# leducthanhig/image-restoration-models

Hardware: AMD Instinct MI355X
Metric: images/sec + PSNR, Restormer motion-deblur 1280x720 (higher is better)
Workload: dtype f32 (1x1 convs: fp32 emulated by 3 fp16 MFMAs on hi/lo operand splits with fp32 accumulation, error vs float64 at the level of an fp32 chain; everything else exact f32; value_exact_f32: f32 MFMA everywhere); 1 GPU; Restormer motion-deblur (WithBias LN, 26.13M params, synthetic weights seed 42) on 1280x720x3 uint8 GoPro-shaped synthetic frames; 6 tiles 512x512 (overlap 96) per frame; a step = 4 frame(s) per GPU, their 24 tiles in one batched forward; global_batch=4, tile=512, overlap=96, parallelism=per-image shard x1, no data-path collective

## Files before the change

image-restoration-models_amd/_hip.py:

```python
from __future__ import annotations

import ctypes as C
import os

import torch

_HERE = os.path.dirname(os.path.abspath(__file__))
LIB_PATH = os.path.join(_HERE, "libirm_hip.so")

ACT_NONE, ACT_RELU, ACT_GELU, ACT_SILU, ACT_RELU6 = 0, 1, 2, 3, 4
LN_NONE, LN_WITHBIAS, LN_BIASFREE = 0, 1, 2

_P, _L, _I, _F, _D = C.c_void_p, C.c_long, C.c_int, C.c_float, C.c_double

SIGNATURES = {
    "irm_version": [],
    "irm_ln_stats_f32": [_P, _L, _P, _I, _I, _I, _F, _P],
    "irm_gemm1x1_f32": [_P, _L, _P, _L, _P, _L, _P, _L, _P, _P, _P, _P, _I, _I, _I, _I, _I, _I, _I, _I, _P, _F, _P, _P],
    "irm_gemm1x1_f16x3_f32": [_P, _L, _P, _L, _P, _L, _P, _L, _P, _P, _P, _P, _I, _I, _I, _I, _I, _I, _I, _I, _P, _F, _P, _P],
    "irm_ln_split_f16": [_P, _L, _P, _P, _I, _F, _F, _P, _I, _I, _I, _P],
    "irm_ln_gemm_presplit_f16x3_f32": [_P, _P, _L, _P, _P, _I, _F, _F, _P, _L, _P, _F, _I, _I, _I, _I, _I, _P],
    "irm_ln_gemm_presplit_cl_f16x3_f32": [_P, _P, _L, _P, _P, _I, _F, _F, _P, _L, _P, _F, _I, _I, _I, _I, _I, _I, _P],
    "irm_gdfn_tail_f16x3_f32": [_P, _L, _P, _P, _P, _P, _L, _F, _I, _I, _I, _I, _I, _I, _P],
    "irm_gemm_presplit_f16x3_f32": [_P, _P, _P, _L, _P, _F, _I, _I, _I, _I, _I, _I, _I, _I, _P],
# ... 40 lines not shown
}

SIGNATURES_HALF = {
    "irm_conv3x3_h_in_f32": [_P, _P, _L, _P, _L, _P, _I, _I, _I, _I, _I, _I, _P],
    "irm_conv3x3_h_f16": [_P, _F, _P, _L, _P, _L, _P, _L, _P, _I, _I, _I, _I, _I, _I, _I, _I, _P],
    "irm_conv3x3_h_out_f32": [_P, _P, _L, _P, _L, _P, _L, _P, _I, _I, _I, _I, _I, _I, _P],
}

SIGNATURES_FRAMES = {
    "irm_frame_minmax_f32": [_P, _L, _P, _P, _L, _P],
    "irm_tile_extract_f32": [_P, _P, _P, _P, _P, _I, _I, _I, _I, _I, _I, _I, _I, _I, _P],
    "irm_window_blend_f32": [_P, _P, _P, _P, _P, _I, _I, _I, _I, _I, _I, _I, _I, _I, _I, _I, _P],
}

SIGNATURES_GRAM = {
    "irm_dw_gram_cm_f16x3_f32": [_P, _L, _P, _P, _P, _P, _I, _I, _I, _I, _I, _P],
}

SIGNATURES_YUV = {
    "irm_yuv420_to_rgb_f32": [_P, _P, _P, _I, _L, _L, _I, _I, _I, _I, _I, _I, _I, _I, _P, _P],
    "irm_rgb_f32_to_yuv420": [_P, _P, _P, _P, _I, _L, _L, _I, _I, _I, _I, _I, _I, _I, _I, _P],
}

SIGNATURES_INCEPTION = {
    "irm_convkxk_f32": [_P, _P, _L, _P, _L, _P, _L, _P, _I, _I, _I, _I, _I, _I, _I, _I, _I, _I, _I, _I, _I, _I, _I, _P],
    "irm_pool3x3_f32": [_P, _L, _P, _L, _I, _I, _I, _I, _I, _P],
}

SIGNATURES_METRICS = {
    "irm_frame_metrics_f32": [_P, _P, _I, _I, _I, _I, _D, _P, _P, _P, _L, _P],
    "irm_yuv420_metrics": [_P, _P, _P, _I, _L, _L, _P, _P, _P, _I, _L, _L, _I, _I, _I, _I, _I, _P, _P, _P, _L, _P],
}

_lib = None


class HipLibraryError(RuntimeError):
    pass


def load():
    global _lib, LIB_PATH
    if _lib is None:
        if os.environ.get("IRM_HIP_LIB"):
            LIB_PATH = os.path.abspath(os.environ["IRM_HIP_LIB"])
        if not os.path.exists(LIB_PATH):
            raise HipLibraryError(
                f"{LIB_PATH} not found: build it with `python -c 'import __graft_entry__ as g; g.build()'` "
                "(make -C image-restoration-models_amd/csrc).  There is no CPU fallback.")
        lib = C.CDLL(LIB_PATH)
        for name, argtypes in {**SIGNATURES, **SIGNATURES_HALF, **SIGNATURES_FRAMES, **SIGNATURES_GRAM,
                               **SIGNATURES_YUV, **SIGNATURES_INCEPTION, **SIGNATURES_METRICS}.items():
            fn = getattr(lib, name)
            fn.argtypes = argtypes
            fn.restype = _I
        _lib = lib
    return _lib


def _stream() -> int:
    return torch.cuda.current_stream().cuda_stream


def ptr(t):
    if t is None:
        return None
    if isinstance(t, int):
        return t
    assert t.is_cuda, "HIP kernels need device tensors"
    return t.data_ptr()


def call(name: str, *args):
    rc = getattr(load(), name)(*args, _stream())
    if rc != 0:
        raise HipLibraryError(f"{name} failed with status {rc} "
                              f"({'invalid arguments' if rc == -1 else 'HIP launch error'})")



def pack_gemm_weight(w: torch.Tensor) -> torch.Tensor:
    w = w.detach().reshape(w.shape[0], -1).float()
    m, k = w.shape
    mt, ks = (m + 15) // 16, 4 * ((k + 15) // 16)
    wpad = torch.zeros(mt * 16, ks * 4, dtype=torch.float32, device=w.device)
# ... 420 lines not shown
```

image-restoration-models_amd/csrc/conv3x3_f16.hip:

```cpp
#include "conv_epilogue.h"


#define CF_TH 8
#define CF_TW IRM_CONV_TW
#define CF_PLANE 400
#define CF_HC 34
#define CF_NP 340
#define CF_PXB 160
#define CF_RAWB (7 * 512 * 16)
#define CF_IMGB (CF_NP * CF_PXB)
#define CF_NRAW 7


__device__ __forceinline__ float cf_res(float v, float r, int mode) {
    if (mode == 1) return v + r;
    if (mode == 2) return r - v;
    return fminf(fmaxf(tanhf(v) + r, -1.0f), 1.0f);
}

struct ConvF16Args {
    const float* Wp;
    const float* X; long x_bs;
    float* Y; long y_bs;
    const float* R; long r_bs;
    const float* bias;
    int Ci, Co, H, W, mtiles, S;
    int relu1, res_mode, relu2, store_mode, tiles_x;
    float inv_s;
    float slope;
    int ps_r;
};


template <int CT, int NCH = 1>
__global__ __launch_bounds__(512, 2) void conv3x3_f16x3_kernel(ConvF16Args a) {
    constexpr int TT = CT * NCH;
    constexpr int NG = 3 * NCH;
    constexpr int WGB = 3 * CT * 2048;
    constexpr int NW = (WGB / 16 + 511) / 512;
    extern __shared__ __attribute__((aligned(16))) float smem[];
    char* lds = reinterpret_cast<char*>(smem);
    char* raw = lds;
    char* img = lds + CF_RAWB;
    char* wbuf = img + CF_IMGB;

    const int tid = threadIdx.x, lane = tid & 63, wave = __builtin_amdgcn_readfirstlane(tid >> 6);
    const int g = lane >> 4, r = lane & 15;
    const int b = blockIdx.z;
    const int ty0 = (blockIdx.x / a.tiles_x) * CF_TH, tx0 = (blockIdx.x % a.tiles_x) * CF_TW;
    const float* X = a.X + (long)b * a.x_bs;
    const long plane = (long)a.H * a.W;
    const int S = a.S;
    const int nchunks = (a.mtiles + TT - 1) / TT;
    const int my_chunks = (nchunks - (int)blockIdx.y + (int)gridDim.y - 1) / (int)gridDim.y;

    long xoff[CF_NRAW];
    int xch[CF_NRAW];
    bool xok[CF_NRAW];
#pragma unroll
    for (int j = 0; j < CF_NRAW; ++j) {
        const int q = j * 512 + tid;
        const int ch = q / 100, rem = q - ch * 100, row = rem / 10, chunk = rem - row * 10;
        const int gy = ty0 - 1 + row, gx = tx0 - 4 + chunk * 4;
        xch[j] = ch;
        xok[j] = q < 3200 && gy >= 0 && gy < a.H && gx >= 0 && gx < a.W;
        xoff[j] = (long)ch * plane + (long)gy * a.W + gx;
    }
    const float* const zero_page = irm_zero_page;
// ... 78 lines not shown
                        const int pi = (wave + dy) * CF_HC + 16 * p + r + dx;
                        ah[p] = *reinterpret_cast<const irm_h8*>(img + pi * CF_PXB + 16 * g);
                        al[p] = *reinterpret_cast<const irm_h8*>(img + pi * CF_PXB + 64 + 16 * g);
                    }
#pragma unroll
                    for (int c = 0; c < CT; ++c) {
                        const irm_h8 wh = *reinterpret_cast<const irm_h8*>(wb + ((c * 3 + tl) * 2) * 1024 + lane * 16);
                        const irm_h8 wl = *reinterpret_cast<const irm_h8*>(wb + ((c * 3 + tl) * 2 + 1) * 1024 + lane * 16);
#pragma unroll
                        for (int p = 0; p < 2; ++p) {
                            f32x4& t = acc[p][chn * CT + c];
                            t = irm_mfma3_f16(ah[p], al[p], wh, wl, t);
                        }
                    }
                }
            }
        }
#pragma unroll
        for (int c = 0; c < TT; ++c) {
            const int co = (mt0 + c) * 16 + r;
            const bool row_ok = mt0 + c < a.mtiles && co < a.Co;
            const float bv = (a.bias && row_ok) ? a.bias[co] : 0.0f;
#pragma unroll
            for (int p = 0; p < 2; ++p) {
                const int y = ty0 + wave, x = tx0 + p * 16 + g * 4;
                float v[4];
#pragma unroll
                for (int e = 0; e < 4; ++e) {
                    v[e] = fmaf(acc[p][c][e], a.inv_s, bv);
                    if (a.relu1 == 1) v[e] = fmaxf(v[e], 0.0f);
                    else if (a.relu1 == 2) v[e] = v[e] > 0.0f ? v[e] : v[e] * a.slope;
                }
                if (!row_ok || y >= a.H || x >= a.W) continue;
                if (a.store_mode == 0) {
                    const long off = (long)co * plane + (long)y * a.W + x;
                    if (a.res_mode) {
                        const float4 rr = *reinterpret_cast<const float4*>(R + off);
                        const float rv[4] = {rr.x, rr.y, rr.z, rr.w};
#pragma unroll
                        for (int e = 0; e < 4; ++e) v[e] = cf_res(v[e], rv[e], a.res_mode);
                    }
                    if (a.relu2) {
#pragma unroll
                        for (int e = 0; e < 4; ++e) v[e] = fmaxf(v[e], 0.0f);
                    }
                    *reinterpret_cast<float4*>(Y + off) = make_float4(v[0], v[1], v[2], v[3]);
                } else if (a.store_mode == 1) {
                    const int oh = a.H >> 1, ow = a.W >> 1;
                    const long op = (long)oh * ow;
                    const int oc = co * 4 + (y & 1) * 2;
                    const long o = (long)(y >> 1) * ow + (x >> 1);
                    *reinterpret_cast<float2*>(Y + (long)oc * op + o) = make_float2(v[0], v[2]);
                    *reinterpret_cast<float2*>(Y + (long)(oc + 1) * op + o) = make_float2(v[1], v[3]);
                } else if (a.ps_r == 2) {
                    const int ow = a.W * 2;
                    const long op = (long)a.H * 2 * ow;
                    const int oc = co >> 2, i = (co >> 1) & 1, jx = co & 1;
                    float* o = Y + (long)oc * op + (long)(2 * y + i) * ow + 2 * x + jx;
#pragma unroll
                    for (int e = 0; e < 4; ++e) o[2 * e] = v[e];
                } else {
                    const int pr = a.ps_r, ow = a.W * pr;
                    const long op = (long)a.H * pr * ow;
                    const int oc = co / (pr * pr), i = (co / pr) % pr, jx = co % pr;
                    float* o = Y + (long)oc * op + (long)(pr * y + i) * ow + pr * x + jx;
#pragma unroll
                    for (int e = 0; e < 4; ++e) o[pr * e] = v[e];
                }
            }
        }
    }
}

template <int CT, int NCH = 1>
static int launch_conv_f16(const ConvF16Args& a, int B, int ygroups, hipStream_t stream) {
    const size_t lds = (size_t)CF_RAWB + CF_IMGB + 2 * (3 * CT * 2048);
    static_assert((size_t)CF_RAWB + CF_IMGB + 2 * (3 * CT * 2048) <= 160 * 1024, "LDS");
    IRM_ALLOW_BIG_LDS((&conv3x3_f16x3_kernel<CT, NCH>));
    const int tiles_y = (a.H + CF_TH - 1) / CF_TH;
    dim3 grid(a.tiles_x * tiles_y, ygroups, B);
    hipLaunchKernelGGL((conv3x3_f16x3_kernel<CT, NCH>), grid, dim3(512), lds, stream, a);
    return irm_launch_status();
}

extern "C" int irm_conv3x3_f16x3_ep_f32(const float* wp_split, float inv_scale, const float* x, long x_bs, float* y,
                                        long y_bs, const float* res, long r_bs, const float* bias, int B, int Ci, int Co,
                                        int H, int W, int act1, float slope, int res_mode, int relu2, int store_mode,
                                        int shuffle, int ct, int ygroups, hipStream_t stream) {
    ConvF16Args a;
    if (int rc = irm_conv_common(a, wp_split, x, x_bs, y, y_bs, res, r_bs, bias, B, Ci, Co, H, W, act1, slope, res_mode,
                                 relu2, store_mode, shuffle, ct, ygroups)) return rc;
    if ((W & 3) || (x_bs & 3) || (y_bs & 3) || (r_bs & 3)) return IRM_EINVAL;
    if (!irm_aligned16(x) || !irm_aligned16(y) || !irm_aligned16(res) || !irm_aligned16(wp_split)) return IRM_EINVAL;
    a.S = (Ci + 31) / 32; a.inv_s = inv_scale;
    switch (ct) {
        case 1: return launch_conv_f16<1>(a, B, ygroups, stream);
        case 2: return launch_conv_f16<2>(a, B, ygroups, stream);
        case 3: return launch_conv_f16<3>(a, B, ygroups, stream);
        case 4: return launch_conv_f16<4>(a, B, ygroups, stream);
        case 8: return launch_conv_f16<4, 2>(a, B, ygroups, stream);
        case 12: return launch_conv_f16<4, 3>(a, B, ygroups, stream);
        default: return IRM_EINVAL;
    }
}

extern "C" int irm_conv3x3_f16x3_f32(const float* wp_split, float inv_scale, const float* x, long x_bs, float* y, long y_bs,
                                     const float* res, long r_bs, const float* bias, int B, int Ci, int Co, int H, int W,
                                     int relu1, int res_mode, int relu2, int store_mode, int ct, int ygroups,
                                     hipStream_t stream) {
    return irm_conv3x3_f16x3_ep_f32(wp_split, inv_scale, x, x_bs, y, y_bs, res, r_bs, bias, B, Ci, Co, H, W, relu1 ? 1 : 0,
                                    0.0f, res_mode, relu2, store_mode, 2, ct, ygroups, stream);
}
```

image-restoration-models_amd/csrc/elementwise.hip:

```cpp
#include "irm_common.h"

template <bool VEC, int PQ>
__global__ __launch_bounds__(256) void ln_stats_kernel(const float* __restrict__ x, long x_bs,
                                                       float* __restrict__ stats, int C, int N, float eps) {
    constexpr int G = 256 / PQ;
    __shared__ float4 pm[G][PQ], pq[G][PQ], ps[G][PQ];
    const int b = blockIdx.y;
    const int q = threadIdx.x % PQ, g = threadIdx.x / PQ;
    const int n = (blockIdx.x * PQ + q) * 4;
    const float* p = x + (long)b * x_bs;
    float4 mean = make_float4(0.f, 0.f, 0.f, 0.f), m2 = mean, sum = mean;
    int cnt = 0;
    auto push = [&](const float4& v) {
        sum.x += v.x; sum.y += v.y; sum.z += v.z; sum.w += v.w;
        const float rc = 1.0f / (float)(++cnt);
        float d;
        d = v.x - mean.x; mean.x += d * rc; m2.x += d * (v.x - mean.x);
        d = v.y - mean.y; mean.y += d * rc; m2.y += d * (v.y - mean.y);
        d = v.z - mean.z; mean.z += d * rc; m2.z += d * (v.z - mean.z);
        d = v.w - mean.w; mean.w += d * rc; m2.w += d * (v.w - mean.w);
    };
    if (n < N) {
        int c = g;
        for (; c + 3 * G < C; c += 4 * G) {
// ... 180 lines not shown
#pragma unroll
        for (int i = 0; i < 6; ++i) { a0[i] = a1[i]; a1[i] = a2[i]; }
    }
}

static int dw_launch(bool gate, const DwArgs& a, int B, hipStream_t stream) {
    constexpr int RS = 8;
    const long total = (long)a.C * ((a.H + RS - 1) / RS) * ((a.W + 3) >> 2);
    const long blocks = (total + 255) / 256;
    if (blocks > 2147483647L || B > 65535) return IRM_EINVAL;
    dim3 grid((unsigned)blocks, B);
    const bool vec = !(a.W & 3) && !(a.x_bs & 3) && !(a.y_bs & 3) && irm_aligned16(a.x) && irm_aligned16(a.y);
    if (gate && vec) hipLaunchKernelGGL((dwconv3x3_kernel<true, RS, true>), grid, dim3(256), 0, stream, a);
    else if (gate) hipLaunchKernelGGL((dwconv3x3_kernel<true, RS, false>), grid, dim3(256), 0, stream, a);
    else if (vec) hipLaunchKernelGGL((dwconv3x3_kernel<false, RS, true>), grid, dim3(256), 0, stream, a);
    else hipLaunchKernelGGL((dwconv3x3_kernel<false, RS, false>), grid, dim3(256), 0, stream, a);
    return irm_launch_status();
}

extern "C" int irm_dwconv3x3_f32(const float* x, long x_bs, const float* w, const float* bias, float* y,
                                 long y_bs, int B, int C, int H, int W, int act, hipStream_t stream) {
    if (!x || !w || !y || B <= 0 || C <= 0 || H <= 0 || W <= 0) return IRM_EINVAL;
    if (act < 0 || act > 3) return IRM_EINVAL;
    DwArgs a{x, x_bs, w, bias, y, y_bs, C, H, W, act};
    return dw_launch(false, a, B, stream);
}

extern "C" int irm_dwconv3x3_gate_f32(const float* x, long x_bs, const float* w, const float* bias, float* y,
                                      long y_bs, int B, int hid, int H, int W, hipStream_t stream) {
    if (!x || !w || !y || B <= 0 || hid <= 0 || H <= 0 || W <= 0) return IRM_EINVAL;
    DwArgs a{x, x_bs, w, bias, y, y_bs, hid, H, W, IRM_ACT_NONE};
    return dw_launch(true, a, B, stream);
}
```

image-restoration-models_amd/ops.py:

```python
from __future__ import annotations

import os

import torch

from . import _hip
from ._hip import ACT_GELU, ACT_NONE, ACT_RELU, ACT_RELU6, ACT_SILU, LN_BIASFREE, LN_NONE, LN_WITHBIAS


class KernelTimer:

    def __init__(self, detail=False, only=None):
        self.records = []
        self.detail = detail
        self.only = None if only is None else frozenset(only)
        self._chain = {}
        self._done = {}
        self._since = 0

    def _fold(self, k, e0, e1, fl, by):
        d = self._done.setdefault(k, dict(launches=0, ms=0.0, flops=0.0, bytes=0.0))
        d["launches"] += 1
        d["ms"] += e0.elapsed_time(e1)
        d["flops"] += fl
# ... 407 lines not shown
        ygroups = max(1, min(nchunks, -(-target_blocks() // blocks)))
    return ct, ygroups


def conv3x3(wp, x, y, ci: int, co: int, *, bias=None, relu1=False, res=None, res_mode=0, relu2=False,
            store_mode=0, ct: int | None = None, ygroups: int | None = None, leaky: float | None = None, shuffle: int = 2):
    _chk(x, "x"), _chk(y, "y")
    B, _, H, W = x.shape
    nbytes = 4.0 * B * H * W * (ci + co + (co if res is not None else 0))
    if leaky is not None and relu1:
        raise ValueError("conv3x3: relu1 and leaky are exclusive")
    act1, slope = (2, float(leaky)) if leaky is not None else (int(bool(relu1)), 0.0)
    extra = (f" ps{shuffle}" if shuffle != 2 else "") + (f" leaky{slope:g}" if leaky is not None else "")
    if isinstance(wp, _hip.ConvWeight):
        aligned = (W % 4 == 0 and _bs(x) % 4 == 0 and _bs(y) % 4 == 0 and _bs(res) % 4 == 0 and x.data_ptr() % 16 == 0
                   and y.data_ptr() % 16 == 0 and (res is None or res.data_ptr() % 16 == 0))
        if wp.raw is not None and aligned and store_mode == 0 and act1 < 2:
            _launch("conv3x3_thin", 18.0 * B * ci * co * H * W, nbytes, "irm_conv3x3_thin_f32", _hip.ptr(wp.raw), _hip.ptr(x),
                    _bs(x), _hip.ptr(y), _bs(y), _hip.ptr(res), _bs(res), _hip.ptr(bias), B, ci, co, H, W, int(relu1),
                    int(res_mode), int(relu2), tag=f"ci{ci} co{co} {H}x{W} B{B}")
            return
        wp = (wp.split, wp.inv_scale) if (wp.split is not None and aligned) else wp.exact
    if isinstance(wp, tuple):
        kernel, entry, lead = "conv3x3_f16x3", "irm_conv3x3_f16x3_ep_f32", (_hip.ptr(wp[0]), float(wp[1]))
    else:
        kernel, entry, lead = "conv3x3", "irm_conv3x3_ep_f32", (_hip.ptr(wp),)
    ct, ygroups = plan_conv3x3(co, H, W, B, split=isinstance(wp, tuple), ct=ct, ygroups=ygroups)
    _launch(kernel, 18.0 * B * ci * co * H * W, nbytes, entry, *lead, _hip.ptr(x), _bs(x), _hip.ptr(y), _bs(y),
            _hip.ptr(res), _bs(res), _hip.ptr(bias), B, ci, co, H, W, act1, slope, int(res_mode), int(relu2),
            int(store_mode), int(shuffle), ct, ygroups,
            tag=f"ci{ci} co{co} {H}x{W} B{B} ct{ct} yg{ygroups} st{store_mode}{extra}")


def transpose(src: torch.Tensor, dst: torch.Tensor, R: int, C: int):
    B = src.shape[0]
    _launch("transpose", 0.0, 8.0 * B * R * C, "irm_transpose_f32", _hip.ptr(src), src.stride(0), _hip.ptr(dst),
            dst.stride(0), B, R, C, tag=f"R{R} C{C} B{B}")


def scan_is_flat(D: int, N: int, R: int) -> bool:
    return (N, R) in ((1, 4), (16, 4)) and D % 64 != 0


def scan_plan(B: int, L: int, D: int, flat: bool = False):
    DB = (D + 63) // 64
    waves = -(-4 * D // 64) if flat else 4 * DB
    nchunk = max(1, min(-(-L // 32), -(-3072 // (B * waves))))
    chunk = max(32, -(-(-(-L // nchunk)) // 8) * 8)
    return chunk, -(-L // chunk), DB


def selective_scan(xT, pT, ids, dtw, dtb, A, Dskip, yT, state, sdt, ysum, B, L, D, N, R, chunk):
    flops = B * 4.0 * L * D * (2 * R + 9 * N + 12)
    nbytes = 4.0 * B * L * (D + 4 * (R + 2 * N) + 4 * D)
    _launch("selective_scan", flops, nbytes, "irm_selective_scan_f32", _hip.ptr(xT), _hip.ptr(pT), _hip.ptr(ids),
            _hip.ptr(dtw), _hip.ptr(dtb), _hip.ptr(A), _hip.ptr(Dskip), _hip.ptr(yT), _hip.ptr(state), _hip.ptr(sdt),
            _hip.ptr(ysum), B, L, D, N, R, chunk, tag=f"L{L} D{D} N{N} B{B} chunk{chunk}")


def losh_combine(ysum, gw, gb, gate, yT, nw, nb, z, out, B, L, D, nchunk, eps=1e-5):
    _chk(z, "z"), _chk(out, "out")
    _launch("losh_combine", 12.0 * B * L * D, 4.0 * B * L * D * 6, "irm_losh_combine_f32", _hip.ptr(ysum), _hip.ptr(gw),
            _hip.ptr(gb), _hip.ptr(gate), _hip.ptr(yT), _hip.ptr(nw), _hip.ptr(nb), _hip.ptr(z), _bs(z), _hip.ptr(out),
            _bs(out), B, L, D, nchunk, float(eps), tag=f"L{L} D{D} B{B}")


# ... 62 lines not shown
```

image-restoration-models_amd/restormer/restormer.py:

```python
from __future__ import annotations

import os

import torch
import torch.nn as nn

from .. import _hip, ops, unet
from ..host import ModelHost, f32

SYNTH_RULES = (
    (r"^output\.weight$", "gain", 0.02),
    (r"^skip_conv\.weight$", "gain", 0.5),
)


def _hidden(dim, factor):
    return int(dim * factor)


class _Norm(nn.Module):

    def __init__(self, dim, kind):
        super().__init__()
        self.body = nn.Module()
# ... 118 lines not shown

    def __init__(self, inp_channels=3, out_channels=3, dim=48, num_blocks=(4, 6, 6, 8),
                 num_refinement_blocks=4, heads=(1, 2, 4, 8), ffn_expansion_factor=2.66, bias=False,
                 LayerNorm_type="WithBias", dual_pixel_task=False):
        super().__init__()
        f, ln = ffn_expansion_factor, LayerNorm_type
        d1, d2, d3, d4 = dim, dim * 2, dim * 4, dim * 8
        self.inp_channels, self.out_channels, self.dim = inp_channels, out_channels, dim
        self.patch_embed = _Proj(inp_channels, d1, bias=False)
        self.encoder_level1 = _stage(d1, heads[0], num_blocks[0], f, bias, ln)
        self.down1_2 = _Resample(d1, d1 // 2)
        self.encoder_level2 = _stage(d2, heads[1], num_blocks[1], f, bias, ln)
        self.down2_3 = _Resample(d2, d2 // 2)
        self.encoder_level3 = _stage(d3, heads[2], num_blocks[2], f, bias, ln)
        self.down3_4 = _Resample(d3, d3 // 2)
        self.latent = _stage(d4, heads[3], num_blocks[3], f, bias, ln)
        self.up4_3 = _Resample(d4, d4 * 2)
        self.reduce_chan_level3 = nn.Conv2d(d4, d3, 1, bias=bias)
        self.decoder_level3 = _stage(d3, heads[2], num_blocks[2], f, bias, ln)
        self.up3_2 = _Resample(d3, d3 * 2)
        self.reduce_chan_level2 = nn.Conv2d(d3, d2, 1, bias=bias)
        self.decoder_level2 = _stage(d2, heads[1], num_blocks[1], f, bias, ln)
        self.up2_1 = _Resample(d2, d2 * 2)
        self.decoder_level1 = _stage(d2, heads[0], num_blocks[0], f, bias, ln)
        self.refinement = _stage(d2, heads[0], num_refinement_blocks, f, bias, ln)
        self.dual_pixel_task = dual_pixel_task
        if dual_pixel_task:
            self.skip_conv = nn.Conv2d(d1, d2, 1, bias=bias)
        self.output = nn.Conv2d(d2, out_channels, 3, padding=1, bias=bias)
        self._split = False
        self.max_tiles_per_batch = 12
        self.hip_graph = True
        self._tap = None

    def _build(self):
        self._split = not os.environ.get("IRM_GEMM_EXACT")
        pk = {name: pack_block(m, self._split) for name, m in self.named_modules() if isinstance(m, TransformerBlock)}
        pk.update(unet.pack_unet(self))
        for name in ("reduce_chan_level3", "reduce_chan_level2"):
            if self._split and _hip.split_is_safe(getattr(self, name).weight):
                pk[name + "_s"] = _hip.pack_gemm_weight_split(getattr(self, name).weight)
        return pk

    def _block(self, blk: TransformerBlock, w: dict, x: torch.Tensor, have_stats: bool = False,
               want_stats: bool = True) -> bool:
        B, C, H, W = x.shape
        N = H * W
        dev = x.device
        heads = blk.attn.num_heads
        hid = blk.ffn.hidden
        fuse = ops.can_fuse_stats(C)
        stats = self._buf("stats", B * 2 * N, dev)
        big_a = self._buf("scratch_a", B * max(3 * C, 2 * hid) * N, dev)
        big_b = self._buf("scratch_b", B * max(3 * C, hid) * N, dev)
        qkv = big_a[:B * 3 * C * N].view(B, 3 * C, H, W)
        qkv2 = big_b[:B * 3 * C * N].view(B, 3 * C, H, W)
        split = self._split and N % 4 == 0
        s_qkv, s_pin, s_pout = split and "qkv_s" in w, split and "pin_s" in w, split and "pout_s" in w
        s_fold = split and w.get("mfold_split", False)
        presplit = split and "qkv_ps" in w and ops.can_presplit(C, N)
        if presplit:
            xs = self._buf("xsplit", B * C * N, dev)
            frag, out_scale, s_x = w["qkv_ps"]
            ops.ln_gemm_presplit(frag, x, qkv, 3 * C, C, w["n1w"], w["n1b"], blk.norm1.mode, s_x, out_scale=out_scale,
                                 bias=w["qkv_b"], xs=xs)
        else:
# ... 59 lines not shown
        N = H * W
        dev = x.device
        heads, hid = blk.attn.num_heads, blk.ffn.hidden
        qkv = self._buf("scratch_a", B * 3 * C * N, dev).view(B, 3 * C, H, W)
        tm = ops.can_qk_tile_major(C, heads, H, W)
        fa = "gdfn_fa" in w
        assert not (x_tm or y_tm) or (tm and fa), "tile-major x / y: only between the kernels that understand them"
        v_tm = tm and fa
        gram_in_qkv = tm and "gram_s" in w and ops.can_qkv_gram(C, heads, H, W)
        nchunk, rec = ops.gram_part_plan(B, C, heads, H, W, tiled=gram_in_qkv)
        nready = None
        part = self._buf("gram_part", B * heads * nchunk * rec, dev)
        if gram_in_qkv:
            nready = ops.qkv_gram_cm(w["qkv_f"], x, qkv, w["gram_s"], part, C, ln_mode=blk.norm1.mode, x_tm=x_tm, v_tm=v_tm)
        else:
            ops.qkv_dw_fused(w["qkv_f"], x, qkv, C, 3 * C, ln_mode=blk.norm1.mode, tm=tm, x_tm=x_tm, v_tm=v_tm)
        gsum = self._buf("gram_sum", B * heads * rec, dev)
        mfold_n = ops.mfold_numel(C)
        mfold = self._zeros(("mfold", C, B), B * mfold_n, dev)
        s_fold = w.get("mfold_split", False)
        if fa:
            mfrag = self._zeros(("mfold_frag", C, B), B * ops.mfold_frag_numel(C), dev)
            ops.mdta_fold(qkv, part, gsum, w["temp"], w["wout"], mfrag, C, heads, gram_scale=w.get("gram_s"), frag=True, tm=tm,
                          nchunk_ready=nready)
            ops.attn_gdfn_fused(w["gdfn_fa"], x, qkv[:, 2 * C:], mfrag, alt, C, hid, ln_mode=blk.norm2.mode,
                                bias_o=w["wout_b"], bias=w["pout_b"], x_tm=x_tm, v_tm=v_tm, y_tm=y_tm)
            return alt
        ops.mdta_fold(qkv, part, gsum, w["temp"], w["wout"], mfold, C, heads, split=s_fold, gram_scale=w.get("gram_s"), tm=tm,
                      nchunk_ready=nready)
        ops.gemm1x1(mfold, qkv[:, 2 * C:], x, C, C, res=x, bias=w["wout_b"], w_bs=mfold_n, split=s_fold)
        ops.gdfn_fused(w["gdfn_f"], x, alt, C, hid, ln_mode=blk.norm2.mode, bias=w["pout_b"])
        return alt

    def _run_stage(self, name, pk, x, have_stats=False):
        names = (name,) if isinstance(name, str) else tuple(name)
        blocks = [(f"{n}.{i}", blk) for n in names for i, blk in enumerate(getattr(self, n))]
        B, C, H, W = x.shape
        if (len(blocks) and all("gdfn_f" in pk[k] for k, _ in blocks) and ops.can_fuse_gdfn(C, W) and (H * W) % 4 == 0
                and len({blk.attn.num_heads for _, blk in blocks}) == 1):
            cur, alt = x, self._buf(f"alt_{C}", B * C * H * W, x.device).view(B, C, H, W)
            heads = blocks[0][1].attn.num_heads
            act_tm = all("gdfn_fa" in pk[k] for k, _ in blocks) and ops.can_qk_tile_major(C, heads, H, W)
            for i, (k, blk) in enumerate(blocks):
                out = self._block_fused(blk, pk[k], cur, alt, x_tm=act_tm and i > 0, y_tm=act_tm and i + 1 < len(blocks))
                cur, alt = out, cur
            if cur is not x:
                x.copy_(cur)
                if ops.TIMER is not None:
                    ops.TIMER.break_chain()
            return False
        for n in names:
            stage = getattr(self, n)
            for i, blk in enumerate(stage):
                have_stats = self._block(blk, pk[f"{n}.{i}"], x, have_stats, want_stats=i + 1 < len(stage))
        return have_stats

    @torch.no_grad()
    def forward(self, inp_img: torch.Tensor) -> torch.Tensor:
        self._require_cuda(inp_img)
        x = inp_img.float().contiguous()
        if x.shape[2] % 8 or x.shape[3] % 8:
            raise ValueError("Restormer needs H and W to be multiples of 8 (the tiler pads, utils.pad)")
        pk = self._pack()
        tap = self.__dict__.get("_tap")
        return unet.forward(self, x, pk, lambda names, t, level: self._run_stage(names, pk, t),
                            None if tap is None else lambda t: tap.__setitem__("refinement", t.clone()))
```

image-restoration-models_amd/unet.py:

```python
from __future__ import annotations

import torch

from . import _hip, ops
from .host import f32

RESAMPLE = ("down1_2", "down2_3", "down3_4", "up4_3", "up3_2", "up2_1")


def pack_unet(model) -> dict:
    pk = {name: _hip.pack_conv3x3(getattr(model, name).body[0].weight) for name in RESAMPLE}
    pk["patch_embed"] = _hip.pack_conv3x3(model.patch_embed.proj.weight)
    pk["output"] = _hip.pack_conv3x3(model.output.weight)
    pk["output_b"] = f32(model.output.bias)
    for name in ("reduce_chan_level3", "reduce_chan_level2") + (("skip_conv",) if model.dual_pixel_task else ()):
        pk[name] = _hip.pack_gemm_weight(getattr(model, name).weight)
        pk[name + "_b"] = f32(getattr(model, name).bias)
    return pk


def _reduce_chan(pk, name, cat, dec, c):
    split = name + "_s" in pk and (cat.shape[2] * cat.shape[3]) % 4 == 0
    ops.gemm1x1(pk[name + "_s" if split else name], cat, dec, c, 2 * c, bias=pk[name + "_b"], split=split)


def forward(model, x, pk, run_stage, after_trunk=None):
    B, Cin, H, W = x.shape
    dev = x.device
    d1, d2, d3, d4 = model.dim, model.dim * 2, model.dim * 4, model.dim * 8
    H2, W2, H3, W3, H4, W4 = H // 2, W // 2, H // 4, W // 4, H // 8, W // 8

    def buf(name, ch, h, w):
        return model._buf(name, B * ch * h * w, dev).view(B, ch, h, w)

    cat1 = buf("cat1", 2 * d1, H, W)
    cat2 = buf("cat2", 2 * d2, H2, W2)
    cat3 = buf("cat3", 2 * d3, H3, W3)
    lat = buf("latent", d4, H4, W4)
    dec3 = buf("dec3", d3, H3, W3)
    dec2 = buf("dec2", d2, H2, W2)

    e1 = cat1[:, d1:]
    ops.conv3x3(pk["patch_embed"], x, e1, Cin, d1)
    if model.dual_pixel_task:
        e1_in = buf("enc1_in", d1, H, W)
        e1_in.copy_(e1)
        if ops.TIMER is not None:
            ops.TIMER.break_chain()
    run_stage(("encoder_level1",), e1, 0)
    e2 = cat2[:, d2:]
    ops.conv3x3(pk["down1_2"], e1, e2, d1, d1 // 2, store_mode=1)
    run_stage(("encoder_level2",), e2, 1)
    e3 = cat3[:, d3:]
    ops.conv3x3(pk["down2_3"], e2, e3, d2, d2 // 2, store_mode=1)
    run_stage(("encoder_level3",), e3, 2)
    ops.conv3x3(pk["down3_4"], e3, lat, d3, d3 // 2, store_mode=1)
    run_stage(("latent",), lat, 3)

    ops.conv3x3(pk["up4_3"], lat, cat3[:, :d3], d4, d4 * 2, store_mode=2)
    _reduce_chan(pk, "reduce_chan_level3", cat3, dec3, d3)
    run_stage(("decoder_level3",), dec3, 2)
    ops.conv3x3(pk["up3_2"], dec3, cat2[:, :d2], d3, d3 * 2, store_mode=2)
    _reduce_chan(pk, "reduce_chan_level2", cat2, dec2, d2)
    run_stage(("decoder_level2",), dec2, 1)
    ops.conv3x3(pk["up2_1"], dec2, cat1[:, :d1], d2, d2 * 2, store_mode=2)
    run_stage(("decoder_level1", "refinement"), cat1, 0)
    if after_trunk is not None:
        after_trunk(cat1)

    out = torch.empty(B, model.out_channels, H, W, dtype=torch.float32, device=dev)
    if model.dual_pixel_task:
        ops.gemm1x1(pk["skip_conv"], e1_in, cat1, d2, d1, res=cat1, bias=pk["skip_conv_b"])
        ops.conv3x3(pk["output"], cat1, out, d2, model.out_channels, bias=pk["output_b"])
    else:
        ops.conv3x3(pk["output"], cat1, out, d2, model.out_channels, bias=pk["output_b"], res=x, res_mode=1)
    return out
```

include/irm_hip.h:

```cpp
#ifndef IRM_HIP_H
#define IRM_HIP_H

#ifdef __cplusplus
extern "C" {
#endif

typedef struct ihipStream_t* irm_stream_t;

#define IRM_OK 0
#define IRM_EINVAL (-1)
#define IRM_ELAUNCH (-2)

#define IRM_ACT_NONE 0
#define IRM_ACT_RELU 1
#define IRM_ACT_GELU 2
#define IRM_ACT_SILU 3

#define IRM_LN_NONE 0
#define IRM_LN_WITHBIAS 1
#define IRM_LN_BIASFREE 2

int irm_version(void);

int irm_ln_stats_f32(const float* x, long x_bs, float* stats, int B, int C, int N, float eps,
// ... 132 lines not shown
int irm_dwconv3x3_s2_f32(const float* x, long x_bs, const float* w, float* y, long y_bs, int B, int C, int H, int W,
                         irm_stream_t stream);
int irm_upsample_add_f32(const float* src, long s_bs, const float* add, long a_bs, float* out, long o_bs, int B, int C,
                         int Hs, int Ws, int scale, irm_stream_t stream);

int irm_dihedral_chop_f32(const float* src, const int* table, float* dst, long dst_pixels, int B, int C, int H, int W,
                          int P, int max_ph, int max_pw, irm_stream_t stream);
int irm_ensemble_merge_f32(const float* pred, const int* table, float* out, long pred_pixels, int B, int Co, int H,
                           int W, int P, int scale, irm_stream_t stream);

int irm_transpose_f32(const float* in, long in_bs, float* out, long out_bs, int B, int R, int C,
                      irm_stream_t stream);

int irm_selective_scan_f32(const float* xT, const float* pT, const int* ids, const float* dtw, const float* dtb,
                           const float* A, const float* Dskip, float* yT, float* state, float* sdt, float* ysum,
                           int B, int L, int D, int N, int R, int chunk, irm_stream_t stream);

int irm_losh_combine_f32(float* ysum, const float* gw, const float* gb, float* gate, const float* yT,
                         const float* nw, const float* nb, const float* z, long z_bs, float* out, long out_bs,
                         int B, int L, int D, int nchunk, float eps, irm_stream_t stream);

#include "irm_hip_half.h"

#include "irm_hip_frames.h"

#include "irm_hip_gram.h"

#include "irm_hip_yuv.h"

#include "irm_hip_inception.h"

#include "irm_hip_metrics.h"

#ifdef __cplusplus
}
#endif
#endif
```

Baseline: 22.34 images/s.

## Store down/up-sample conv outputs tile-major to enter fused stages without relayout

```diff
diff --git a/image-restoration-models_amd/_hip.py b/image-restoration-models_amd/_hip.py
--- a/image-restoration-models_amd/_hip.py
+++ b/image-restoration-models_amd/_hip.py
@@ -96,6 +96,11 @@
     "irm_yuv420_metrics": [_P, _P, _P, _I, _L, _L, _P, _P, _P, _I, _L, _L, _I, _I, _I, _I, _I, _P, _P, _P, _L, _P],
 }
 
+SIGNATURES_STAGE = {
+    "irm_conv3x3_f16x3_tm_f32": [_P, _F, _P, _L, _P, _L, _P, _I, _I, _I, _I, _I, _I, _I, _I, _I, _I, _P],
+    "irm_planar_to_tm_f32": [_P, _L, _P, _L, _I, _I, _I, _I, _I, _I, _P],
+}
+
 _lib = None
 
 
@@ -114,7 +119,8 @@
                 "(make -C image-restoration-models_amd/csrc).  There is no CPU fallback.")
         lib = C.CDLL(LIB_PATH)
         for name, argtypes in {**SIGNATURES, **SIGNATURES_HALF, **SIGNATURES_FRAMES, **SIGNATURES_GRAM,
-                               **SIGNATURES_YUV, **SIGNATURES_INCEPTION, **SIGNATURES_METRICS}.items():
+                               **SIGNATURES_YUV, **SIGNATURES_INCEPTION, **SIGNATURES_METRICS,
+                               **SIGNATURES_STAGE}.items():
             fn = getattr(lib, name)
             fn.argtypes = argtypes
             fn.restype = _I
diff --git a/image-restoration-models_amd/csrc/conv3x3_f16.hip b/image-restoration-models_amd/csrc/conv3x3_f16.hip
--- a/image-restoration-models_amd/csrc/conv3x3_f16.hip
+++ b/image-restoration-models_amd/csrc/conv3x3_f16.hip
@@ -32,8 +32,8 @@
 };
 
 
-template <int CT, int NCH = 1>
-__global__ __launch_bounds__(512, 2) void conv3x3_f16x3_kernel(ConvF16Args a) {
+template <int CT, int NCH = 1, bool TM = false, class Args = ConvF16Args>
+__global__ __launch_bounds__(512, 2) void conv3x3_f16x3_kernel(Args a) {
     constexpr int TT = CT * NCH;
     constexpr int NG = 3 * NCH;
     constexpr int WGB = 3 * CT * 2048;
@@ -178,6 +178,22 @@
                     else if (a.relu1 == 2) v[e] = v[e] > 0.0f ? v[e] : v[e] * a.slope;
                 }
                 if (!row_ok || y >= a.H || x >= a.W) continue;
+                if constexpr (TM) {
+                    const long cb = a.tm_cb;
+                    if (a.store_mode == 1) {
+                        const int oy = y >> 1, ox = x >> 1, otx = a.W >> 6;
+                        const int oc = co * 4 + (y & 1) * 2;
+                        float* o = Y + (((long)(oy >> 3) * otx + (ox >> 5)) * 256 + (oy & 7) * 32 + (ox & 31)) * cb + oc;
+                        *reinterpret_cast<float2*>(o) = make_float2(v[0], v[1]);
+                        *reinterpret_cast<float2*>(o + cb) = make_float2(v[2], v[3]);
+                    } else {
+                        const int oy = 2 * y + ((co >> 1) & 1), ox = 2 * x + (co & 1), otx = a.W >> 4;
+                        float* o = Y + (((long)(oy >> 3) * otx + (ox >> 5)) * 256 + (oy & 7) * 32 + (ox & 31)) * cb + (co >> 2);
+#pragma unroll
+                        for (int e = 0; e < 4; ++e) o[2 * e * cb] = v[e];
+                    }
+                    continue;
+                }
                 if (a.store_mode == 0) {
                     const long off = (long)co * plane + (long)y * a.W + x;
                     if (a.res_mode) {
@@ -218,6 +234,10 @@
     }
 }
 
+struct ConvF16TmArgs : ConvF16Args {
+    int tm_cb;
+};
+
 template <int CT, int NCH = 1>
 static int launch_conv_f16(const ConvF16Args& a, int B, int ygroups, hipStream_t stream) {
     const size_t lds = (size_t)CF_RAWB + CF_IMGB + 2 * (3 * CT * 2048);
@@ -226,6 +246,16 @@
     const int tiles_y = (a.H + CF_TH - 1) / CF_TH;
     dim3 grid(a.tiles_x * tiles_y, ygroups, B);
     hipLaunchKernelGGL((conv3x3_f16x3_kernel<CT, NCH>), grid, dim3(512), lds, stream, a);
+    return irm_launch_status();
+}
+
+template <int CT, int NCH = 1>
+static int launch_conv_f16_tm(const ConvF16TmArgs& a, int B, int ygroups, hipStream_t stream) {
+    const size_t lds = (size_t)CF_RAWB + CF_IMGB + 2 * (3 * CT * 2048);
+    IRM_ALLOW_BIG_LDS((&conv3x3_f16x3_kernel<CT, NCH, true, ConvF16TmArgs>));
+    const int tiles_y = (a.H + CF_TH - 1) / CF_TH;
+    dim3 grid(a.tiles_x * tiles_y, ygroups, B);
+    hipLaunchKernelGGL((conv3x3_f16x3_kernel<CT, NCH, true, ConvF16TmArgs>), grid, dim3(512), lds, stream, a);
     return irm_launch_status();
 }
 
@@ -250,6 +280,31 @@
     }
 }
 
+extern "C" int irm_conv3x3_f16x3_tm_f32(const float* wp_split, float inv_scale, const float* x, long x_bs, float* y,
+                                        long y_bs, const float* bias, int B, int Ci, int Co, int H, int W, int store_mode,
+                                        int Cb, int c_off, int ct, int ygroups, hipStream_t stream) {
+    ConvF16TmArgs a;
+    if (store_mode != 1 && store_mode != 2) return IRM_EINVAL;
+    if (int rc = irm_conv_common(a, wp_split, x, x_bs, y, y_bs, nullptr, 0, bias, B, Ci, Co, H, W, 0, 0.0f, 0, 0, store_mode,
+                                 2, ct, ygroups)) return rc;
+    if ((W & 3) || (x_bs & 3) || (y_bs & 3)) return IRM_EINVAL;
+    if (!irm_aligned16(x) || !irm_aligned16(y) || !irm_aligned16(wp_split)) return IRM_EINVAL;
+    if (store_mode == 1 ? ((H & 15) || (W & 63)) : ((H & 3) || (W & 15))) return IRM_EINVAL;
+    const long co_out = store_mode == 1 ? 4L * Co : Co / 4;
+    if (Cb <= 0 || (Cb & 3) || (c_off & 3) || c_off < 0 || c_off + co_out > Cb) return IRM_EINVAL;
+    a.S = (Ci + 31) / 32; a.inv_s = inv_scale;
+    a.Y = y + c_off; a.tm_cb = Cb;
+    switch (ct) {
+        case 1: return launch_conv_f16_tm<1>(a, B, ygroups, stream);
+        case 2: return launch_conv_f16_tm<2>(a, B, ygroups, stream);
+        case 3: return launch_conv_f16_tm<3>(a, B, ygroups, stream);
+        case 4: return launch_conv_f16_tm<4>(a, B, ygroups, stream);
+        case 8: return launch_conv_f16_tm<4, 2>(a, B, ygroups, stream);
+        case 12: return launch_conv_f16_tm<4, 3>(a, B, ygroups, stream);
+        default: return IRM_EINVAL;
+    }
+}
+
 extern "C" int irm_conv3x3_f16x3_f32(const float* wp_split, float inv_scale, const float* x, long x_bs, float* y, long y_bs,
                                      const float* res, long r_bs, const float* bias, int B, int Ci, int Co, int H, int W,
                                      int relu1, int res_mode, int relu2, int store_mode, int ct, int ygroups,
diff --git a/image-restoration-models_amd/csrc/elementwise.hip b/image-restoration-models_amd/csrc/elementwise.hip
--- a/image-restoration-models_amd/csrc/elementwise.hip
+++ b/image-restoration-models_amd/csrc/elementwise.hip
@@ -236,3 +236,42 @@
     DwArgs a{x, x_bs, w, bias, y, y_bs, hid, H, W, IRM_ACT_NONE};
     return dw_launch(true, a, B, stream);
 }
+
+#define PT_CC 48
+#define PT_LD 260
+
+__global__ __launch_bounds__(256) void planar_to_tm_kernel(const float* __restrict__ x, long x_bs, float* __restrict__ y,
+                                                           long y_bs, int C, int H, int W, int Cb, int c_off) {
+    __shared__ __attribute__((aligned(16))) float lds[PT_CC * PT_LD];
+    const int tid = threadIdx.x;
+    const int tiles_x = W >> 5;
+    const int ty = blockIdx.x / tiles_x, tx = blockIdx.x - ty * tiles_x;
+    const int c0 = blockIdx.y * PT_CC, nc = min(PT_CC, C - c0);
+    const long plane = (long)H * W;
+    const float* xb = x + (long)blockIdx.z * x_bs + (long)c0 * plane + (long)(ty * 8) * W + tx * 32;
+    for (int i = tid; i < nc * 64; i += 256) {
+        const int c = i >> 6, r = (i >> 3) & 7, q = i & 7;
+        const float4 v = *reinterpret_cast<const float4*>(xb + (long)c * plane + (long)r * W + 4 * q);
+        *reinterpret_cast<float4*>(lds + c * PT_LD + r * 32 + 4 * q) = v;
+    }
+    __syncthreads();
+    const int n4 = nc >> 2;
+    float* yb = y + (long)blockIdx.z * y_bs + (long)blockIdx.x * 256 * Cb + c_off + c0;
+    for (int i = tid; i < 256 * n4; i += 256) {
+        const int p = i / n4, j = i - p * n4;
+        const float* s = lds + (4 * j) * PT_LD + p;
+        *reinterpret_cast<float4*>(yb + (long)p * Cb + 4 * j) = make_float4(s[0], s[PT_LD], s[2 * PT_LD], s[3 * PT_LD]);
+    }
+}
+
+extern "C" int irm_planar_to_tm_f32(const float* x, long x_bs, float* y, long y_bs, int B, int C, int H, int W, int Cb,
+                                    int c_off, hipStream_t stream) {
+    if (!x || !y || B <= 0 || C <= 0 || H <= 0 || W <= 0 || B > 65535) return IRM_EINVAL;
+    if ((H & 7) || (W & 31) || (C & 3) || (Cb & 3) || (c_off & 3) || c_off < 0 || (long)c_off + C > Cb) return IRM_EINVAL;
+    if ((x_bs & 3) || (y_bs & 3) || !irm_aligned16(x) || !irm_aligned16(y)) return IRM_EINVAL;
+    const long tiles = (long)(H >> 3) * (W >> 5);
+    if (tiles > 2147483647L || (C + PT_CC - 1) / PT_CC > 65535) return IRM_EINVAL;
+    dim3 grid((unsigned)tiles, (C + PT_CC - 1) / PT_CC, B);
+    hipLaunchKernelGGL(planar_to_tm_kernel, grid, dim3(256), 0, stream, x, x_bs, y, y_bs, C, H, W, Cb, c_off);
+    return irm_launch_status();
+}
diff --git a/image-restoration-models_amd/ops.py b/image-restoration-models_amd/ops.py
--- a/image-restoration-models_amd/ops.py
+++ b/image-restoration-models_amd/ops.py
@@ -463,6 +463,41 @@
             tag=f"ci{ci} co{co} {H}x{W} B{B} ct{ct} yg{ygroups} st{store_mode}{extra}")
 
 
+def can_conv3x3_tm(wp, ci: int, co: int, H: int, W: int, store_mode: int) -> bool:
+    if not isinstance(wp, _hip.ConvWeight) or wp.split is None:
+        return False
+    if store_mode == 1:
+        return H % 16 == 0 and W % 64 == 0
+    return store_mode == 2 and co % 4 == 0 and H % 4 == 0 and W % 16 == 0
+
+
+def conv3x3_tm(wp, x, y, ci: int, co: int, *, store_mode: int, c_off: int = 0, bias=None, ct: int | None = None,
+               ygroups: int | None = None):
+    _chk(x, "x"), _chk(y, "y")
+    B, _, H, W = x.shape
+    Cb = y.shape[1]
+    if not can_conv3x3_tm(wp, ci, co, H, W, store_mode):
+        raise ValueError(f"conv3x3_tm: no tile-major store for ci {ci} co {co} {H}x{W} store_mode {store_mode}")
+    oc, oh, ow = (4 * co, H // 2, W // 2) if store_mode == 1 else (co // 4, 2 * H, 2 * W)
+    assert tuple(y.shape[2:]) == (oh, ow) and y.shape[0] == B and c_off % 4 == 0 and 0 <= c_off and c_off + oc <= Cb
+    assert x.data_ptr() % 16 == 0 and y.data_ptr() % 16 == 0 and _bs(x) % 4 == 0 and _bs(y) % 4 == 0
+    nbytes = 4.0 * B * H * W * (ci + co)
+    ct, ygroups = plan_conv3x3(co, H, W, B, split=True, ct=ct, ygroups=ygroups)
+    _launch("conv3x3_f16x3", 18.0 * B * ci * co * H * W, nbytes, "irm_conv3x3_f16x3_tm_f32", _hip.ptr(wp.split),
+            float(wp.inv_scale), _hip.ptr(x), _bs(x), _hip.ptr(y), _bs(y), _hip.ptr(bias), B, ci, co, H, W, int(store_mode),
+            Cb, int(c_off), ct, ygroups, tag=f"ci{ci} co{co} {H}x{W} B{B} ct{ct} yg{ygroups} st{store_mode} tm")
+
+
+def planar_to_tm(x, y, *, c_off: int = 0):
+    _chk(x, "x"), _chk(y, "y")
+    B, C, H, W = x.shape
+    Cb = y.shape[1]
+    assert tuple(y.shape[2:]) == (H, W) and y.shape[0] == B and H % 8 == 0 and W % 32 == 0
+    assert C % 4 == 0 and Cb % 4 == 0 and c_off % 4 == 0 and 0 <= c_off and c_off + C <= Cb
+    _launch("planar_to_tm", 0.0, 8.0 * B * C * H * W, "irm_planar_to_tm_f32", _hip.ptr(x), _bs(x), _hip.ptr(y), _bs(y), B, C, H,
+            W, Cb, int(c_off), tag=f"C{C} {H}x{W} B{B} Cb{Cb}")
+
+
 def transpose(src: torch.Tensor, dst: torch.Tensor, R: int, C: int):
     B = src.shape[0]
     _launch("transpose", 0.0, 8.0 * B * R * C, "irm_transpose_f32", _hip.ptr(src), src.stride(0), _hip.ptr(dst),
diff --git a/image-restoration-models_amd/restormer/restormer.py b/image-restoration-models_amd/restormer/restormer.py
--- a/image-restoration-models_amd/restormer/restormer.py
+++ b/image-restoration-models_amd/restormer/restormer.py
@@ -174,6 +174,10 @@
         self.max_tiles_per_batch = 12
         self.hip_graph = True
         self._tap = None
+        self.stage_entry_tm = True
+
+    def mode_key(self):
+        return super().mode_key() + (bool(self.stage_entry_tm),)
 
     def _build(self):
         self._split = not os.environ.get("IRM_GEMM_EXACT")
@@ -299,23 +303,43 @@
         ops.gdfn_fused(w["gdfn_f"], x, alt, C, hid, ln_mode=blk.norm2.mode, bias=w["pout_b"])
         return alt
 
-    def _run_stage(self, name, pk, x, have_stats=False):
+    def _stage_blocks(self, name):
         names = (name,) if isinstance(name, str) else tuple(name)
-        blocks = [(f"{n}.{i}", blk) for n in names for i, blk in enumerate(getattr(self, n))]
+        return names, [(f"{n}.{i}", blk) for n in names for i, blk in enumerate(getattr(self, n))]
+
+    def _stage_fused(self, blocks, pk, C, H, W):
+        return (len(blocks) and all("gdfn_f" in pk[k] for k, _ in blocks) and ops.can_fuse_gdfn(C, W) and (H * W) % 4 == 0
+                and len({blk.attn.num_heads for _, blk in blocks}) == 1)
+
+    def _stage_act_tm(self, blocks, pk, C, H, W):
+        return (all("gdfn_fa" in pk[k] for k, _ in blocks)
+                and ops.can_qk_tile_major(C, blocks[0][1].attn.num_heads, H, W))
+
+    def _entry_tm(self, name, pk, C, H, W):
+        _, blocks = self._stage_blocks(name)
+        return bool(self.stage_entry_tm and self._stage_fused(blocks, pk, C, H, W) and self._stage_act_tm(blocks, pk, C, H, W))
+
+    def _run_stage(self, name, pk, x, have_stats=False, src=None):
+        names, blocks = self._stage_blocks(name)
         B, C, H, W = x.shape
-        if (len(blocks) and all("gdfn_f" in pk[k] for k, _ in blocks) and ops.can_fuse_gdfn(C, W) and (H * W) % 4 == 0
-                and len({blk.attn.num_heads for _, blk in blocks}) == 1):
+        if self._stage_fused(blocks, pk, C, H, W):
             cur, alt = x, self._buf(f"alt_{C}", B * C * H * W, x.device).view(B, C, H, W)
-            heads = blocks[0][1].attn.num_heads
-            act_tm = all("gdfn_fa" in pk[k] for k, _ in blocks) and ops.can_qk_tile_major(C, heads, H, W)
+            act_tm = self._stage_act_tm(blocks, pk, C, H, W)
+            assert src is None or act_tm, "a tile-major stage entry needs the tile-major chain"
+            if src is not None and src.data_ptr() != x.data_ptr():
+                assert src.shape == x.shape
+                cur = src
             for i, (k, blk) in enumerate(blocks):
-                out = self._block_fused(blk, pk[k], cur, alt, x_tm=act_tm and i > 0, y_tm=act_tm and i + 1 < len(blocks))
+                last = i + 1 == len(blocks)
+                out = self._block_fused(blk, pk[k], cur, x if last and cur is not x else alt,
+                                        x_tm=act_tm and (i > 0 or src is not None), y_tm=act_tm and not last)
                 cur, alt = out, cur
             if cur is not x:
                 x.copy_(cur)
                 if ops.TIMER is not None:
                     ops.TIMER.break_chain()
             return False
+        assert src is None, "a tile-major stage entry needs the fused chain"
         for n in names:
             stage = getattr(self, n)
             for i, blk in enumerate(stage):
@@ -330,5 +354,6 @@
             raise ValueError("Restormer needs H and W to be multiples of 8 (the tiler pads, utils.pad)")
         pk = self._pack()
         tap = self.__dict__.get("_tap")
-        return unet.forward(self, x, pk, lambda names, t, level: self._run_stage(names, pk, t),
-                            None if tap is None else lambda t: tap.__setitem__("refinement", t.clone()))
+        return unet.forward(self, x, pk, lambda names, t, level, src=None: self._run_stage(names, pk, t, src=src),
+                            None if tap is None else lambda t: tap.__setitem__("refinement", t.clone()),
+                            entry_tm=lambda names, C, H, W: self._entry_tm(names, pk, C, H, W))
diff --git a/image-restoration-models_amd/unet.py b/image-restoration-models_amd/unet.py
--- a/image-restoration-models_amd/unet.py
+++ b/image-restoration-models_amd/unet.py
@@ -24,7 +24,10 @@
     ops.gemm1x1(pk[name + "_s" if split else name], cat, dec, c, 2 * c, bias=pk[name + "_b"], split=split)
 
 
-def forward(model, x, pk, run_stage, after_trunk=None):
+def forward(model, x, pk, run_stage, after_trunk=None, entry_tm=None):
+    def tm(names, c, h, w, conv):
+        return entry_tm is not None and entry_tm(names, c, h, w) and ops.can_conv3x3_tm(*conv)
+
     B, Cin, H, W = x.shape
     dev = x.device
     d1, d2, d3, d4 = model.dim, model.dim * 2, model.dim * 4, model.dim * 8
@@ -49,8 +52,12 @@
             ops.TIMER.break_chain()
     run_stage(("encoder_level1",), e1, 0)
     e2 = cat2[:, d2:]
-    ops.conv3x3(pk["down1_2"], e1, e2, d1, d1 // 2, store_mode=1)
-    run_stage(("encoder_level2",), e2, 1)
+    if tm(("encoder_level2",), d2, H2, W2, (pk["down1_2"], d1, d1 // 2, H, W, 1)):
+        ops.conv3x3_tm(pk["down1_2"], e1, e2, d1, d1 // 2, store_mode=1)
+        run_stage(("encoder_level2",), e2, 1, e2)
+    else:
+        ops.conv3x3(pk["down1_2"], e1, e2, d1, d1 // 2, store_mode=1)
+        run_stage(("encoder_level2",), e2, 1)
     e3 = cat3[:, d3:]
     ops.conv3x3(pk["down2_3"], e2, e3, d2, d2 // 2, store_mode=1)
     run_stage(("encoder_level3",), e3, 2)
@@ -63,8 +70,14 @@
     ops.conv3x3(pk["up3_2"], dec3, cat2[:, :d2], d3, d3 * 2, store_mode=2)
     _reduce_chan(pk, "reduce_chan_level2", cat2, dec2, d2)
     run_stage(("decoder_level2",), dec2, 1)
-    ops.conv3x3(pk["up2_1"], dec2, cat1[:, :d1], d2, d2 * 2, store_mode=2)
-    run_stage(("decoder_level1", "refinement"), cat1, 0)
+    if tm(("decoder_level1", "refinement"), d2, H, W, (pk["up2_1"], d2, d2 * 2, H2, W2, 2)):
+        cat1_tm = buf("cat1_tm", 2 * d1, H, W)
+        ops.conv3x3_tm(pk["up2_1"], dec2, cat1_tm, d2, d2 * 2, store_mode=2)
+        ops.planar_to_tm(e1, cat1_tm, c_off=d1)
+        run_stage(("decoder_level1", "refinement"), cat1, 0, cat1_tm)
+    else:
+        ops.conv3x3(pk["up2_1"], dec2, cat1[:, :d1], d2, d2 * 2, store_mode=2)
+        run_stage(("decoder_level1", "refinement"), cat1, 0)
     if after_trunk is not None:
         after_trunk(cat1)
 
diff --git a/include/irm_hip.h b/include/irm_hip.h
--- a/include/irm_hip.h
+++ b/include/irm_hip.h
@@ -188,6 +188,8 @@
 
 #include "irm_hip_metrics.h"
 
+#include "irm_hip_stage.h"
+
 #ifdef __cplusplus
 }
 #endif
diff --git a/include/irm_hip_stage.h b/include/irm_hip_stage.h
--- /dev/null
+++ b/include/irm_hip_stage.h
@@ -0,0 +1,8 @@
+#pragma once
+
+int irm_conv3x3_f16x3_tm_f32(const float* wp_split, float inv_scale, const float* x, long x_bs, float* y, long y_bs,
+                             const float* bias, int B, int Ci, int Co, int H, int W, int store_mode, int Cb, int c_off,
+                             int ct, int ygroups, irm_stream_t stream);
+
+int irm_planar_to_tm_f32(const float* x, long x_bs, float* y, long y_bs, int B, int C, int H, int W, int Cb, int c_off,
+                         irm_stream_t stream);
```

Result: no change. 22.40 images/s (median of 4 runs) (+0.3%).
